# lmdu/pyfastx

Measured on NVIDIA H100. Metric: index_build_GBps, higher is better.
Workload: dtype u8

## Files before the change

### pyfastx_b200/csrc/fxg_scan.cu

```cuda
#include "fxg_common.cuh"
#include <stdlib.h>
#include <string.h>
#include <limits.h>

namespace fxg {

#ifndef FXG_MARK_MINB
#define FXG_MARK_MINB 6
#endif
constexpr int REGION   = 2048;
constexpr int SEGCAP   = 128;
constexpr int MARK_WARPS = 8;
constexpr int PS_THREADS = 256, PS_PER_THREAD = 16, PS_BLOCK = PS_THREADS * PS_PER_THREAD;
constexpr int64_t NOPOS = INT64_MIN / 4;
constexpr uint32_t E_POS = 0x07ffu, E_CR = 1u << 14, E_HDR = 1u << 15;
constexpr uint32_t FW_NF_SHIFT = 11, FW_NF = 3u << FW_NF_SHIFT, FW_GEN = 1u << 13;
constexpr int LF_MAX = 3, LF_STRIDE = 4;
constexpr uint32_t LF_HDR = 0, LF_LLEN = 1, LF_EVENT = 2, LF_CUT_UNKNOWN = 1u << 23;
constexpr uint32_t NAME_SCAN = 64;

struct __align__(16) FastaTmp {
    int64_t  boff;
    int64_t  lineidx;
    int64_t  llen;
// ... 503 lines not shown
        } else if (row < P.qrows_cap) {
            if (ph == 0) {
                int64_t l = len - 1;
                if (l > 0 && cr) --l;
                if (l < 0) l = 0;
                int64_t k = 0;
                if (s + 1 + l + 20 <= P.capacity) {
                    int which;
                    k = find_first_of2(file + s + 1, l, 0x20202020u, 0x00000000u, &which);
                    if (which == 2) k = l;
                } else {
                    for (; k < l; ++k) {
                        const uint8_t ch = file[s + 1 + k];
                        if (ch == 0) { k = l; break; }
                        if (ch == ' ') break;
                    }
                }
                *reinterpret_cast<int2 *>(&P.qrows[row].dlen) = make_int2((int)len, (int)k);
            } else if (ph == 3) {
                P.qrows[row].qoff = P.base_offset + s;
            }
        }
    }
}

template <int MODE>
__device__ __noinline__ Prev2 carry_walk(const ScanParams *Pg, int64_t r) {
    const ScanParams &P = *Pg;
    Prev2 cy;
    const int lane = threadIdx.x & 31;
    cy.pos1 = cy.pos0 = NOPOS; cy.h1 = cy.h0 = 0;
    int need = 2;
    auto push = [&](int64_t pos, uint32_t h) {
        if (need == 2) { cy.pos1 = pos; cy.h1 = h; } else { cy.pos0 = pos; cy.h0 = h; }
        --need;
    };
    int64_t q = r - 1;
    while (need > 0 && q >= 0) {
        const int64_t qq = q - lane;
        const uint32_t c = qq >= 0 ? (P.rc[qq].x & 0xffffu) : 0u;
        const uint32_t nz = __ballot_sync(0xffffffffu, c != 0);
        if (!nz) { q -= 32; continue; }
        const int f = __ffs(nz) - 1;
        q -= f;
        const int cq = (int)__shfl_sync(0xffffffffu, c, f);
        if (cq <= SEGCAP) {
            const uint32_t y = P.rc[q].y;
            push(q * REGION + (int64_t)(y & E_POS), MODE == 0 ? ((y >> 15) & 1u) : 0u);
            if (need > 0 && cq >= 2) push(q * REGION + (int64_t)((y >> 16) & E_POS), MODE == 0 ? (y >> 31) : 0u);
        } else {
            for (int64_t x = q * REGION + REGION - 1; x >= q * REGION && need > 0; --x)
                if (nl_at(P, x)) push(x, is_hdr_at<MODE>(P, x + 1));
        }
        q -= 1;
    }
    if (need > 0) push(-1, is_hdr_at<MODE>(P, 0));
    return cy;
}

template <int MODE>
__device__ __noinline__ unsigned long long dense_region(const ScanParams *Pg, int64_t first_line, int64_t r, Prev2 cy,
                                                        ulonglong2 exv) {
    const ScanParams &P = *Pg;
    unsigned long long my_size = 0;
    const int lane = threadIdx.x & 31;
    const uint8_t *file = P.file;
    const int64_t b0 = r * REGION + lane * 64;
    uint32_t c = 0, h = 0;
    Prev2 inc; inc.pos1 = inc.pos0 = NOPOS; inc.h1 = inc.h0 = 0;
    for (int i = 0; i < 64; ++i) {
        const int64_t x = b0 + i;
        if (nl_at(P, x)) {
            const uint32_t hh = is_hdr_at<MODE>(P, x + 1);
            ++c; h += hh;
            inc.pos0 = inc.pos1; inc.h0 = inc.h1; inc.pos1 = x; inc.h1 = hh;
        }
    }
    uint32_t ic = c, ih = h;
    uint32_t icnt = c > 2 ? 2 : c;
#pragma unroll
    for (int d = 1; d < 32; d <<= 1) {
        const uint32_t oc = __shfl_up_sync(0xffffffffu, ic, d), oh = __shfl_up_sync(0xffffffffu, ih, d);
        const int64_t op1 = shfl_up_i64(inc.pos1, d), op0 = shfl_up_i64(inc.pos0, d);
        const uint32_t oh1 = __shfl_up_sync(0xffffffffu, inc.h1, d), oh0 = __shfl_up_sync(0xffffffffu, inc.h0, d);
        const uint32_t ocnt = __shfl_up_sync(0xffffffffu, icnt, d);
        if (lane >= d) {
            ic += oc; ih += oh;
            if (icnt == 0) { inc.pos1 = op1; inc.h1 = oh1; inc.pos0 = op0; inc.h0 = oh0; icnt = ocnt; }
            else if (icnt == 1 && ocnt >= 1) { inc.pos0 = op1; inc.h0 = oh1; icnt = 2; }
        }
    }
    Prev2 pv;
    pv.pos1 = shfl_up_i64(inc.pos1, 1); pv.pos0 = shfl_up_i64(inc.pos0, 1);
    pv.h1 = __shfl_up_sync(0xffffffffu, inc.h1, 1); pv.h0 = __shfl_up_sync(0xffffffffu, inc.h0, 1);
    uint32_t pcnt = __shfl_up_sync(0xffffffffu, icnt, 1);
    if (lane == 0) pcnt = 0;
    if (pcnt == 0) pv = cy;
    else if (pcnt == 1) { pv.pos0 = cy.pos1; pv.h0 = cy.h1; }
    int64_t idx = (int64_t)exv.x + (ic - c);
    int64_t hcount = (int64_t)exv.y + (ih - h);
    for (int i = 0; i < 64 && c; ++i) {
        const int64_t x = b0 + i;
        if (!nl_at(P, x)) continue;
        const bool cr = x > 0 && file[x - 1] == '\r';
        do_line<MODE>(P, first_line, x, pv.pos1, pv.pos0, pv.h1 != 0, pv.h0 != 0, hcount, idx, cr, my_size);
        const uint32_t hh = is_hdr_at<MODE>(P, x + 1);
        hcount += hh; ++idx;
        pv.pos0 = pv.pos1; pv.h0 = pv.h1; pv.pos1 = x; pv.h1 = hh;
    }
    return my_size;
}

template <int MODE>
__device__ __forceinline__ void region_batches(const ScanParams &P, int64_t first_line, int64_t r, int nl, Prev2 cy, ulonglong2 X,
                                               uint32_t E0, uint32_t E1, unsigned long long &my_size) {
    const int lane = threadIdx.x & 31;
    const uint32_t lt_mask = (1u << lane) - 1u;
    const int64_t base = r * REGION;
    const uint16_t *sg = P.seg + r * SEGCAP;
    int64_t hrun = (int64_t)X.y;
    for (int k0 = 0; k0 < nl; k0 += 32) {
        const int k = k0 + lane;
        const bool valid = k < nl;
        uint32_t e = k0 == 0 ? E0 : (k0 == 32 ? E1 : (valid ? (uint32_t)sg[k] : 0u));
        if (!valid) e = 0;
        const uint32_t hb = __ballot_sync(0xffffffffu, (e & E_HDR) != 0);
        const uint32_t e1 = __shfl_up_sync(0xffffffffu, e, 1), e2 = __shfl_up_sync(0xffffffffu, e, 2);
        if (valid) {
            int64_t pm1, pm2;
            bool h1, h2;
            if (lane >= 1) { pm1 = base + (e1 & E_POS); h1 = (e1 & E_HDR) != 0; } else { pm1 = cy.pos1; h1 = cy.h1 != 0; }
            if (lane >= 2) { pm2 = base + (e2 & E_POS); h2 = (e2 & E_HDR) != 0; }
            else if (lane == 1) { pm2 = cy.pos1; h2 = cy.h1 != 0; }
            else { pm2 = cy.pos0; h2 = cy.h0 != 0; }
            do_line<MODE>(P, first_line, base + (e & E_POS), pm1, pm2, h1, h2, hrun + __popc(hb & lt_mask), (int64_t)X.x + k,
                          (e & E_CR) != 0, my_size);
        }
        const uint32_t l31 = __shfl_sync(0xffffffffu, e, 31), l30 = __shfl_sync(0xffffffffu, e, 30);
        cy.pos1 = base + (l31 & E_POS); cy.h1 = (l31 >> 15) & 1u;
        cy.pos0 = base + (l30 & E_POS); cy.h0 = (l30 >> 15) & 1u;
        hrun += __popc(hb);
    }
}

template <int MODE>
__device__ __noinline__ unsigned long long full_region(const ScanParams *Pg, int64_t first_line, int64_t r, ulonglong2 X) {
    const ScanParams &P = *Pg;
    unsigned long long my_size = 0;
    const int lane = threadIdx.x & 31;
    const int nl = (int)(P.rc[r].x & 0xffffu);
    if (nl == 0) return 0;
    Prev2 cy = carry_walk<MODE>(Pg, r);
    if (MODE != 0) cy.h1 = cy.h0 = 0;
    if (nl <= SEGCAP) region_batches<MODE>(P, first_line, r, nl, cy, X, P.seg[r * SEGCAP + lane], P.seg[r * SEGCAP + 32 + lane], my_size);
    else my_size += dense_region<MODE>(Pg, first_line, r, cy, X);
    return my_size;
}

constexpr int RG = 8;
constexpr int RWIN = RG + 2;
static_assert(RWIN * REGION <= 32768, "window positions must fit 15 bits");

__global__ void __launch_bounds__(MARK_WARPS * 32) fastq_records_kernel(const ScanParams Pin) {
    __shared__ uint16_t s_flat[MARK_WARPS][RWIN * SEGCAP];
    const ScanParams &P = Pin;
    const int64_t first_line = Pin.totals->first_line;
    const int lane = threadIdx.x & 31, warp = threadIdx.x >> 5;
    const int64_t r0 = ((int64_t)blockIdx.x * MARK_WARPS + warp) * RG;
    if (r0 >= P.nreg) return;
    unsigned long long my_size = 0;
    const uint8_t *file = P.file;

    const int64_t rl = r0 - 1 + lane;
    uint2 rec = make_uint2(0u, 0u);
    uint64_t exl = 0;
    if (lane <= RWIN && rl >= 0 && rl < P.nreg) { rec = P.rc[rl]; exl = P.ex[rl].x; }
    const uint32_t nll = rec.x & 0xffffu;
    const uint32_t densem = __ballot_sync(0xffffffffu, nll > (uint32_t)SEGCAP);
    if (densem & (((1u << RG) - 1u) << 1)) {
        for (int i = 0; i < RG; ++i)
            if (r0 + i < P.nreg) my_size += full_region<1>(P.self, first_line, r0 + i, P.ex[r0 + i]);
    } else {
        const uint64_t ex0 = (uint64_t)shfl_i64((int64_t)exl, 1);
        uint16_t *flat = s_flat[warp];
        int W = 0, Ls = 0;
        bool closed = false;
#pragma unroll
        for (int i = 0; i < RWIN; ++i) {
            const int nl = (int)__shfl_sync(0xffffffffu, nll, i + 1);
            if (nl > SEGCAP) closed = true;
            if (!closed) {
                const int k = 2 * lane;
                const uint32_t E2 = k < nl ? reinterpret_cast<const uint32_t *>(P.seg + (r0 + i) * SEGCAP)[lane] : 0u;
                const uint32_t e0 = E2 & 0xffffu, e1 = E2 >> 16;
                if (k < nl) flat[W + k] = (uint16_t)((i * REGION + (int)(e0 & E_POS)) | ((e0 & E_CR) ? 0x8000u : 0u));
                if (k + 1 < nl) flat[W + k + 1] = (uint16_t)((i * REGION + (int)(e1 & E_POS)) | ((e1 & E_CR) ? 0x8000u : 0u));
                if (nl > 64) {
                    const uint16_t *sg = P.seg + (r0 + i) * SEGCAP;
                    for (int kk = 64 + lane; kk < nl; kk += 32) {
                        const uint32_t e = sg[kk];
                        flat[W + kk] = (uint16_t)((i * REGION + (int)(e & E_POS)) | ((e & E_CR) ? 0x8000u : 0u));
                    }
                }
                W += nl;
            }
            if (i == RG - 1) Ls = W;
        }
        __syncwarp();
        int64_t carry;
        {
            const uint32_t pn = __shfl_sync(0xffffffffu, nll, 0), py = __shfl_sync(0xffffffffu, rec.y, 0);
            if (r0 == 0) carry = -1;
            else if (pn >= 1 && pn <= (uint32_t)SEGCAP) carry = (r0 - 1) * REGION + (int64_t)(py & E_POS);
            else carry = carry_walk<1>(P.self, r0).pos1;
        }
        const int64_t span_base = r0 * REGION;
        auto POS = [&](int f) -> int64_t { return f < 0 ? carry : span_base + (int64_t)(flat[f] & 0x7fffu); };
        auto CR = [&](int f) -> bool { return (flat[f] & 0x8000u) != 0; };
        const int64_t g0 = first_line + (int64_t)ex0;
        const int64_t row0 = first_line >> 2;
        int lead = (int)((4 - (g0 & 3)) & 3);
        if (lead > Ls) lead = Ls;
        if (lane < lead) {
            const int f = lane;
            const int64_t g = g0 + f;
            const int ph = (int)(g & 3);
            const int64_t row = (g >> 2) - row0;
            const int64_t pm1 = POS(f - 1), p = POS(f);
            if (ph == 1) {
                const int64_t len = p - pm1 - 1;
                const int64_t rlen = (len > 0 && CR(f)) ? len - 1 : len;
                my_size += (unsigned long long)rlen;
                if (row < P.qrows_cap) { P.qrows[row].soff = P.base_offset + pm1 + 1; P.qrows[row].rlen = rlen; }
            } else if (ph == 3) {
                if (row < P.qrows_cap) P.qrows[row].qoff = P.base_offset + pm1 + 1;
            }
        }
        for (int fb = lead; fb < Ls; fb += 128) {
            const int f = fb + 4 * lane;
            int64_t row = 0, soff = 0, rlen = 0, qoff = 0, len = 0, k = 0;
            bool have1 = false, have3 = false;
            const bool mine = f < Ls;
            if (mine) {
                row = ((g0 + f) >> 2) - row0;
                have1 = f + 1 < W; have3 = f + 3 < W;
                const int64_t pm1 = POS(f - 1), p0 = POS(f);
                len = p0 - pm1 - 1;
                int64_t l = len - 1;
                if (l > 0 && CR(f)) --l;
                if (l < 0) l = 0;
                const int64_t s = pm1 + 1;
                if (s + 1 + l + 20 <= P.capacity) {
                    int which;
                    k = find_first_of2(file + s + 1, l, 0x20202020u, 0x00000000u, &which);
                    if (which == 2) k = l;
                } else {
                    for (; k < l; ++k) {
                        const uint8_t ch = file[s + 1 + k];
                        if (ch == 0) { k = l; break; }
                        if (ch == ' ') break;
                    }
                }
                if (have1) {
                    const int64_t p1 = POS(f + 1);
                    const int64_t len1 = p1 - p0 - 1;
                    soff = P.base_offset + p0 + 1;
                    rlen = (len1 > 0 && CR(f + 1)) ? len1 - 1 : len1;
                    if (f + 1 < Ls) my_size += (unsigned long long)rlen;
                }
                if (have3) qoff = P.base_offset + POS(f + 2) + 1;
            }
            const bool full = mine && have3 && row < P.qrows_cap;
            const int other_full = __shfl_xor_sync(0xffffffffu, full ? 1 : 0, 1);
            const bool pair_full = full && other_full != 0;
            longlong2 a, b;
            a.x = soff; a.y = qoff;
            b.x = rlen; b.y = (long long)(((unsigned long long)(uint32_t)(int)k << 32) | (uint32_t)(int)len);
            const bool odd = (lane & 1) != 0;
            const longlong2 send = odd ? a : b;
            longlong2 recv;
            recv.x = shfl_i64(send.x, lane ^ 1);
            recv.y = shfl_i64(send.y, lane ^ 1);
            if (pair_full) {
                fxg_fastq_row *q0 = &P.qrows[odd ? row - 1 : row];
                reinterpret_cast<longlong2 *>(q0)[odd ? 1 : 0] = odd ? recv : a;
                reinterpret_cast<longlong2 *>(q0 + 1)[odd ? 1 : 0] = odd ? b : recv;
            } else if (mine && row < P.qrows_cap) {
                fxg_fastq_row *q = &P.qrows[row];
                if (have3) {
                    reinterpret_cast<longlong2 *>(q)[0] = a;
                    reinterpret_cast<longlong2 *>(q)[1] = b;
                } else {
                    *reinterpret_cast<int2 *>(&q->dlen) = make_int2((int)len, (int)k);
                    if (have1) { q->soff = soff; q->rlen = rlen; }
                }
            }
        }
    }
#pragma unroll
    for (int d = 16; d > 0; d >>= 1) my_size += (unsigned long long)shfl_down_i64((int64_t)my_size, d);
    if (lane == 0 && my_size) atomicAdd((unsigned long long *)&P.totals->sum_len, my_size);
}

constexpr int ROWS_THREADS = 1024, ROWS_PER_THREAD = PS_BLOCK / ROWS_THREADS;
static_assert(ROWS_PER_THREAD == 4, "one uint4 of first-entry words per thread");

__global__ void __launch_bounds__(ROWS_THREADS) fasta_rows_kernel(const ScanParams P) {
    __shared__ uint32_t s_a[ROWS_THREADS / 32], s_b[ROWS_THREADS / 32];
    const int lane = threadIdx.x & 31, warp = threadIdx.x >> 5;
    const int64_t r0 = (int64_t)blockIdx.x * PS_BLOCK + (int64_t)threadIdx.x * ROWS_PER_THREAD;
    const uint4 qa = reinterpret_cast<const uint4 *>(P.rc + r0)[0], qb = reinterpret_cast<const uint4 *>(P.rc + r0)[1];
    const uint4 fv = *reinterpret_cast<const uint4 *>(P.fw + r0);
    const uint2 rcv[ROWS_PER_THREAD] = {make_uint2(qa.x, qa.y), make_uint2(qa.z, qa.w), make_uint2(qb.x, qb.y), make_uint2(qb.z, qb.w)};
    const uint32_t fwv[ROWS_PER_THREAD] = {fv.x, fv.y, fv.z, fv.w};
    uint2 pv = r0 >= 1 ? P.rc[r0 - 1] : make_uint2(0u, 0u);
    uint32_t a = 0, b = 0;
#pragma unroll
    for (int i = 0; i < ROWS_PER_THREAD; ++i) { a += rcv[i].x & 0xffffu; b += rcv[i].x >> 16; }
    uint32_t ia = a, ib = b;
#pragma unroll
    for (int d = 1; d < 32; d <<= 1) {
        const uint32_t oa = __shfl_up_sync(0xffffffffu, ia, d), ob = __shfl_up_sync(0xffffffffu, ib, d);
        if (lane >= d) { ia += oa; ib += ob; }
    }
    const ulonglong2 bb = P.bs[blockIdx.x];
    if (lane == 31) { s_a[warp] = ia; s_b[warp] = ib; }
    __syncthreads();
    uint32_t wa = 0, wb = 0;
    for (int w = 0; w < warp; ++w) { wa += s_a[w]; wb += s_b[w]; }
    ulonglong2 X = make_ulonglong2(bb.x + wa + ia - a, bb.y + wb + ib - b);
    unsigned long long dummy = 0;
    bool any_general = false;
#pragma unroll
    for (int i = 0; i < ROWS_PER_THREAD; ++i) {
        const int64_t r = r0 + i, base = r * REGION;
        const uint32_t nl = rcv[i].x & 0xffffu, fw = fwv[i], pnl = pv.x & 0xffffu;
        const bool general = nl != 0 && (fw & FW_GEN) != 0;
        const bool walk = nl != 0 && !general && (r == 0 || pnl < 2u || pnl > (uint32_t)SEGCAP);
        Prev2 cy;
        cy.pos1 = base - REGION + (int64_t)(pv.y & E_POS); cy.h1 = (pv.y >> 15) & 1u;
        cy.pos0 = base - REGION + (int64_t)((pv.y >> 16) & E_POS); cy.h0 = pv.y >> 31;
        uint32_t wm = __ballot_sync(0xffffffffu, walk);
        while (wm) {
            const int f = __ffs(wm) - 1;
            wm &= wm - 1u;
            const Prev2 c = carry_walk<0>(P.self, shfl_i64(r, f));
            if (lane == f) cy = c;
        }
        if (general) *reinterpret_cast<ulonglong2 *>(P.lf + r * LF_STRIDE) = X;
        any_general |= general;
        if (nl != 0 && !general) {
            const uint32_t f0 = fw & 0xffffu, f1 = fw >> 16;
            const int64_t p0 = base + (int64_t)(f0 & E_POS);
            do_line<0>(P, 0, p0, cy.pos1, cy.pos0, cy.h1 != 0, cy.h0 != 0, (int64_t)X.y, (int64_t)X.x, false, dummy);
            if (nl >= 2u)
                do_line<0>(P, 0, base + (int64_t)(f1 & E_POS), p0, cy.pos1, (f0 & E_HDR) != 0, cy.h1 != 0,
                           (int64_t)X.y + ((f0 & E_HDR) ? 1 : 0), (int64_t)X.x + 1, false, dummy);
            const uint32_t nf = (fw & FW_NF) >> FW_NF_SHIFT;
            for (uint32_t j = 0; j < nf; ++j) {
                const uint2 lf = P.lf[r * LF_STRIDE + j];
                const int64_t slot = (int64_t)X.y + ((lf.x >> 16) & 31u), lineidx = (int64_t)X.x + ((lf.x >> 11) & 31u);
                if (slot >= P.tmp_cap) continue;
                const uint32_t kind = lf.x >> 21;
                if (kind == LF_HDR) {
                    const int64_t p = base + (int64_t)(lf.x & E_POS), dlen = lf.y & E_POS;
                    const int elen = 1 + (int)((lf.y >> 22) & 1u);
                    const int64_t nlen = (lf.y & LF_CUT_UNKNOWN) ? fasta_name_len(P, p - dlen - elen, dlen) : (int64_t)((lf.y >> 11) & E_POS);
                    fasta_header(P, slot, p, lineidx, dlen, nlen, elen);
                } else if (kind == LF_LLEN) {
                    P.tmp[slot].llen = lf.y;
                } else {
                    fasta_event(P, slot, lineidx, (int32_t)lf.y);
                }
            }
        }
        X.x += nl; X.y += rcv[i].x >> 16;
        pv = rcv[i];
    }
    const int block_general = __syncthreads_or(any_general ? 1 : 0);
    if (threadIdx.x == 0) P.gblk[blockIdx.x] = block_general ? 1u : 0u;
}

__global__ void __launch_bounds__(MARK_WARPS * 32) fasta_general_kernel(const ScanParams P) {
    __shared__ ulonglong2 s_x[MARK_WARPS][32];
    const int lane = threadIdx.x & 31, warp = threadIdx.x >> 5;
    const int64_t R0 = ((int64_t)blockIdx.x * MARK_WARPS + warp) * 32;
    if (R0 >= P.nreg) return;
    const int64_t r = R0 + lane;
    if (!P.gblk[R0 / PS_BLOCK]) return;
    const bool general = r < P.nreg && (P.fw[r] & FW_GEN) != 0;
    if (general) s_x[warp][lane] = *reinterpret_cast<const ulonglong2 *>(P.lf + r * LF_STRIDE);
    uint32_t gm = __ballot_sync(0xffffffffu, general);
    while (gm) {
        const int f = __ffs(gm) - 1;
        gm &= gm - 1u;
        full_region<0>(P.self, 0, R0 + f, s_x[warp][f]);
    }
}

__global__ void __launch_bounds__(256) fasta_finalize_kernel(const FastaTmp *tmp, int64_t tmp_cap, int64_t rows_cap,
                                                             int64_t base_offset, ScanTotals *tot, fxg_fasta_row *rows) {
    int64_t nrows = (int64_t)tot->hdr;
    if (nrows > rows_cap || nrows + 1 > tmp_cap) nrows = 0;
    unsigned long long slen_acc = 0;
    const int64_t stride = (int64_t)gridDim.x * blockDim.x;
    for (int64_t r = (int64_t)blockIdx.x * blockDim.x + threadIdx.x; r < nrows; r += stride) {
        const FastaTmp t = tmp[r + 1];
        int64_t next_h, next_line;
        if (r + 1 < nrows) {
            const FastaTmp nx = tmp[r + 2];
            next_h = nx.boff - (1 + nx.dlen + (int64_t)nx.elen);
            next_line = nx.lineidx;
        } else {
            next_h = base_offset + tot->n_eff;
            next_line = (int64_t)tot->nl;
        }
        const int64_t blen = next_h - t.boff;
        const int64_t nlines = next_line - t.lineidx - 1;
        const int64_t slen = blen - nlines * (int64_t)t.elen;
        int norm;
        if (t.D == 0) norm = 1;
        else if (t.D == 1) norm = ((int64_t)t.evmax == t.lineidx + nlines) ? 1 : 0;
        else if (t.D == 2) norm = ((t.evmax - (~t.evminc) == 1) && t.S == 0) ? 1 : 0;
        else norm = 0;
        fxg_fasta_row o;
        o.boff = t.boff; o.blen = blen; o.slen = slen; o.llen = t.llen;
        o.dlen = t.dlen; o.nlen = t.nlen; o.elen = (uint8_t)t.elen; o.norm = (uint8_t)norm;
        for (int i = 0; i < 6; ++i) o.pad[i] = 0;
        o.pad[0] = (t.D == 0 || (t.D == 1 && (int64_t)t.evmax == t.lineidx + nlines && (int64_t)t.S < 0)) ? 1 : 0;
        rows[r] = o;
        slen_acc += (unsigned long long)slen;
    }
#pragma unroll
    for (int d = 16; d > 0; d >>= 1) slen_acc += (unsigned long long)shfl_down_i64((int64_t)slen_acc, d);
    if ((threadIdx.x & 31) == 0 && slen_acc) atomicAdd((unsigned long long *)&tot->sum_len, slen_acc);
    if (blockIdx.x == 0 && threadIdx.x == 0) {
        const FastaTmp l = tmp[0];
        tot->lead_llen = l.llen;
        if (nrows > 0) {
            const FastaTmp f = tmp[1];
            tot->lead_lines = f.lineidx;
            tot->lead_bytes = f.boff - base_offset - (1 + f.dlen + (int64_t)f.elen);
        }
    }
}

__global__ void __launch_bounds__(32) edge_kernel(const ScanParams P, int mode, fxg_shard_info *info) {
    const int lane = threadIdx.x;
    int found = 0;
    int64_t pos[3] = {0, 0, 0};
    for (int64_t r0 = 0; r0 < P.nreg && found < 3; r0 += 32) {
        const int64_t r = r0 + lane;
        const uint32_t c = r < P.nreg ? (P.rc[r].x & 0xffffu) : 0u;
        uint32_t nz = __ballot_sync(0xffffffffu, c != 0);
        while (nz && found < 3) {
            const int fl = __ffs(nz) - 1;
            nz &= nz - 1;
            const int64_t q = r0 + fl;
            for (int64_t x0 = q * REGION; x0 < q * REGION + REGION && found < 3; x0 += 512) {
                const int64_t x = x0 + lane * 16;
                uint32_t m = 0;
                if (x + 16 <= P.n) {
                    const uint4 v = *reinterpret_cast<const uint4 *>(P.file + x);
                    const uint32_t w[4] = {v.x, v.y, v.z, v.w};
#pragma unroll
                    for (int i = 0; i < 16; ++i) m |= (((w[i >> 2] >> (8 * (i & 3))) & 0xffu) == '\n' ? 1u : 0u) << i;
                } else {
                    for (int i = 0; i < 16; ++i) m |= (nl_at(P, x + i) ? 1u : 0u) << i;
                }
                uint32_t any = __ballot_sync(0xffffffffu, m != 0);
                while (any && found < 3) {
                    const int fl2 = __ffs(any) - 1;
                    any &= any - 1u;
                    uint32_t mm = __shfl_sync(0xffffffffu, m, fl2);
                    while (mm && found < 3) { pos[found++] = x0 + fl2 * 16 + (__ffs(mm) - 1); mm &= mm - 1u; }
                }
            }
        }
    }
    if (lane == 0) {
        const ScanTotals t = *P.totals;
        fxg_shard_info o;
        o.n_rows = mode == 0 ? (int64_t)t.hdr : 0;
        o.n_lines = (int64_t)t.nl;
        o.bytes = P.n;
        o.base_offset = P.base_offset;
        o.end_position = t.n_eff;
        o.edge_n = found;
        int64_t start = 0;
        for (int j = 0; j < 3; ++j) {
            o.edge_off[j] = 0; o.edge_len[j] = 0;
            if (j < found) {
                const int64_t p = pos[j];
                const bool cr = p > start && p - 1 < P.n && P.file[p - 1] == '\r';
                o.edge_off[j] = P.base_offset + start;
                o.edge_len[j] = p - start - (cr ? 1 : 0);
                start = p + 1;
            }
        }
        for (int j = 0; j < 4; ++j) o.reserved[j] = 0;
        *info = o;
    }
}

__global__ void shard_prefix_kernel(const fxg_shard_info *all, int nranks, int rank, int mode, ScanTotals *tot) {
    if (threadIdx.x != 0 || blockIdx.x != 0) return;
    int64_t F = 0, T = 0;
    for (int p = 0; p < nranks; ++p) {
        const int64_t nlp = all[p].n_lines;
        if (p < rank) F += nlp;
        T += nlp;
    }
    if (mode == 0) F = 0;
    tot->first_line = F;
    tot->total_lines = T;
    const int64_t nl = (int64_t)tot->nl;
    tot->nrows = mode == 0 ? (int64_t)tot->hdr : (F + nl + 3) / 4 - F / 4;
    tot->sum_len = 0;
}

__global__ void __launch_bounds__(256) clear_kernel(const ScanParams P, int mode, int64_t tmp_slots) {
    const int64_t nrows = P.totals->nrows;
    const int64_t stride = (int64_t)gridDim.x * blockDim.x;
    const int64_t t0 = (int64_t)blockIdx.x * blockDim.x + threadIdx.x;
    if (mode == 0) {
        int64_t slots = nrows + 2;
        if (slots > tmp_slots) slots = tmp_slots;
        uint4 *p = reinterpret_cast<uint4 *>(P.tmp);
        for (int64_t i = t0; i < slots * 4; i += stride) p[i] = make_uint4(0u, 0u, 0u, 0u);
    } else if (t0 < 4) {
        const int64_t row = t0 < 2 ? 0 : nrows - 1;
        if (row >= 0 && row < P.qrows_cap) reinterpret_cast<uint4 *>(P.qrows + row)[t0 & 1] = make_uint4(0u, 0u, 0u, 0u);
    }
}

__global__ void fastq_stitch_kernel(const ScanParams P, const fxg_shard_info *all, int nranks, int rank) {
    if (threadIdx.x != 0 || blockIdx.x != 0) return;
    ScanTotals *tot = P.totals;
    const int64_t F = tot->first_line, n = (int64_t)tot->nl, T = tot->total_lines;
    const int64_t first_read = (F + 3) / 4;
    int64_t last_read = n > 0 ? (F + n - 1) / 4 : first_read - 1;
    if (last_read > T / 4 - 1) last_read = T / 4 - 1;
    const int64_t owned = last_read >= first_read ? last_read - first_read + 1 : 0;
    tot->row0 = first_read - F / 4;
    tot->n_owned = owned;
    if (owned == 0) return;
    const int64_t row = last_read - F / 4;
    if (row >= P.qrows_cap) return;
    for (int ph = 1; ph <= 3; ph += 2) {
        const int64_t g = 4 * last_read + ph;
        if (g < F + n) continue;
        int64_t Fp = F + n;
        for (int p = rank + 1; p < nranks; ++p) {
            const int64_t np = all[p].n_lines;
            if (g < Fp + np) {
                const int64_t j = g - Fp;
                if (j < all[p].edge_n) {
                    if (ph == 1) { P.qrows[row].soff = all[p].edge_off[j]; P.qrows[row].rlen = all[p].edge_len[j]; }
                    else P.qrows[row].qoff = all[p].edge_off[j];
                }
                break;
            }
            Fp += np;
        }
    }
}

__global__ void __launch_bounds__(256) split_point_kernel(const uint8_t *file, int64_t n, int64_t from, int want_header,
                                                          long long *out) {
    __shared__ long long s_best;
    if (threadIdx.x == 0) s_best = LLONG_MAX;
    __syncthreads();
    if (from <= 0) {
        if (!want_header || (n > 0 && file[0] == '>')) { if (threadIdx.x == 0) *out = 0; return; }
        from = 1;
    }
    for (int64_t c0 = from - 1; c0 < n; c0 += 256 * 16) {
        const int64_t a = c0 + threadIdx.x * 16;
        long long mine = LLONG_MAX;
        for (int i = 0; i < 16; ++i) {
            const int64_t x = a + i;
            if (x < n && file[x] == '\n' && (!want_header || (x + 1 < n && file[x + 1] == '>'))) { mine = x + 1; break; }
        }
        if (mine != LLONG_MAX) atomicMin(&s_best, mine);
        __syncthreads();
        if (s_best != LLONG_MAX) break;
        __syncthreads();
    }
    if (threadIdx.x == 0) *out = s_best == LLONG_MAX ? n : s_best;
}

}

using namespace fxg;

static int64_t guess_rows(int mode, int64_t n) { return (mode == 0 ? n / 1024 : n / 200) + 4096; }

static int scan_params(fxg_ctx *ctx, const fxg_file *f, int mode, int64_t base_offset, int flags, bool reserve,
                       ScanParams *out, int64_t *tmp_slots) {
    const int64_t n = f->size;
    const int64_t nreg = (n + 1 + REGION - 1) / REGION;
    const int64_t nb = (nreg + PS_BLOCK - 1) / PS_BLOCK;
    const int64_t nreg_pad = nb * PS_BLOCK;
    const size_t off_bs = fxg_round_up((int64_t)nreg_pad * 8, 256);
    const size_t off_x = off_bs + fxg_round_up(nb * (int64_t)sizeof(ulonglong2), 256);
    const size_t off_gb = off_x + fxg_round_up(nreg_pad * (int64_t)sizeof(uint32_t), 256);
    const size_t off_lf = off_gb + fxg_round_up(nb * (int64_t)sizeof(uint32_t), 256);
    const size_t tile_bytes = mode == 0 ? off_lf + (size_t)nreg * LF_STRIDE * sizeof(uint2) : off_x + (size_t)nreg * sizeof(ulonglong2);
    int rc;
    if (reserve) {
        if ((rc = ctx->counters.reserve(1024))) return rc;
        if ((rc = ctx->tile_desc.reserve(tile_bytes))) return rc;
        if ((rc = ctx->seg.reserve((size_t)nreg * SEGCAP * sizeof(uint16_t)))) return rc;
        const int64_t want = guess_rows(mode, n);
        if (mode == 0) {
            if (ctx->row_tmp.cap < (size_t)(want + 2) * sizeof(FastaTmp) && (rc = ctx->row_tmp.reserve((size_t)(want + 2) * sizeof(FastaTmp)))) return rc;
            if (ctx->rows.cap < (size_t)(want + 1) * sizeof(fxg_fasta_row) && (rc = ctx->rows.reserve((size_t)(want + 1) * sizeof(fxg_fasta_row)))) return rc;
        } else if (ctx->rows.cap < (size_t)(want + 2) * sizeof(fxg_fastq_row)) {
            if ((rc = ctx->rows.reserve((size_t)(want + 2) * sizeof(fxg_fastq_row)))) return rc;
        }
    }
    ScanParams P;
    memset(&P, 0, sizeof(P));
    P.file = f->d; P.n = n; P.capacity = f->capacity & ~(int64_t)15; P.nreg = nreg;
    P.base_offset = base_offset; P.first_line = 0; P.flags = flags;
    P.rc = (uint2 *)ctx->tile_desc.ptr;
    P.bs = (ulonglong2 *)((uint8_t *)ctx->tile_desc.ptr + off_bs);
    if (mode == 0) {
        P.fw = (uint32_t *)((uint8_t *)ctx->tile_desc.ptr + off_x);
        P.gblk = (uint32_t *)((uint8_t *)ctx->tile_desc.ptr + off_gb);
        P.lf = (uint2 *)((uint8_t *)ctx->tile_desc.ptr + off_lf);
    } else {
        P.ex = (ulonglong2 *)((uint8_t *)ctx->tile_desc.ptr + off_x);
    }
    P.seg = (uint16_t *)ctx->seg.ptr;
    P.totals = (ScanTotals *)((uint8_t *)ctx->counters.ptr + 64);
    *tmp_slots = 0;
    if (mode == 0) {
        *tmp_slots = (int64_t)(ctx->row_tmp.cap / sizeof(FastaTmp));
        P.tmp = (FastaTmp *)ctx->row_tmp.ptr;
        P.tmp_cap = *tmp_slots - 1;
    } else {
        P.qrows = (fxg_fastq_row *)ctx->rows.ptr;
        P.qrows_cap = (int64_t)(ctx->rows.cap / sizeof(fxg_fastq_row));
    }
    *out = P;
    return FXG_OK;
}

static fxg_shard_info *own_info(fxg_ctx *ctx) { return (fxg_shard_info *)((uint8_t *)ctx->counters.ptr + 256); }

extern "C" int fxg_scan_begin(fxg_ctx *ctx, const fxg_file *f, int mode, int64_t base_offset, int flags,
                              fxg_shard_info *d_info_out) {
    FXG_CHECK_ARG(ctx && f && (mode == 0 || mode == 1), "null ctx/file or bad mode");
    FXG_LOCK(ctx);
    FXG_CUDA(cudaSetDevice(ctx->device));
    ctx->run.active = false;
    ScanParams P;
    int64_t tmp_slots;
    int rc = scan_params(ctx, f, mode, base_offset, flags, true, &P, &tmp_slots);
    if (rc) return rc;
    const int64_t n = f->size, nreg = P.nreg;
    const int64_t nb = (nreg + PS_BLOCK - 1) / PS_BLOCK, nreg_pad = nb * PS_BLOCK;
    FXG_CUDA(cudaMemsetAsync(ctx->counters.ptr, 0, 1024, ctx->stream));
    if (nreg_pad > nreg) FXG_CUDA(cudaMemsetAsync(P.rc + nreg, 0, (size_t)(nreg_pad - nreg) * 8, ctx->stream));
    const unsigned grid = (unsigned)((nreg + MARK_WARPS - 1) / MARK_WARPS);
    {
        FxgProfScope prof(ctx, FXG_PROF_SCAN);
        if (mode == 0) mark_kernel<0, 1><<<grid, MARK_WARPS * 32, 0, ctx->stream>>>(P);
        else mark_kernel<1, 2><<<grid, MARK_WARPS * 32, 0, ctx->stream>>>(P);
    }
    FXG_CUDA(cudaGetLastError());
    {
        FxgProfScope prof(ctx, FXG_PROF_PREFIX, mode == 0 ? 3 : 4);
        prefix_reduce_kernel<<<(unsigned)nb, PS_THREADS, 0, ctx->stream>>>(P.rc, P.bs);
        prefix_blocks_kernel<<<1, 1024, 0, ctx->stream>>>(P.bs, nb, P.file, n, mode, P.totals);
        if (mode == 1) prefix_expand_kernel<<<(unsigned)nb, PS_THREADS, 0, ctx->stream>>>(P.rc, P.bs, P.ex, nreg);
        edge_kernel<<<1, 32, 0, ctx->stream>>>(P, mode, own_info(ctx));
    }
    FXG_CUDA(cudaGetLastError());
    if (d_info_out)
        FXG_CUDA(cudaMemcpyAsync(d_info_out, own_info(ctx), sizeof(fxg_shard_info), cudaMemcpyDeviceToDevice, ctx->stream));
    ctx->run.active = true; ctx->run.mode = mode; ctx->run.flags = flags; ctx->run.file = f; ctx->run.base_offset = base_offset;
    return FXG_OK;
}

static int launch_phase_b(fxg_ctx *ctx, const ScanParams &P0, int mode, int64_t tmp_slots, const fxg_shard_info *d_all,
                          int nranks, int rank) {
    int rc0 = ctx->params.reserve(512);
    if (rc0) return rc0;
    if (!ctx->h_counters) FXG_CUDA(cudaHostAlloc(&ctx->h_counters, 8192, cudaHostAllocDefault));
    ScanParams P = P0;
    P.self = (const ScanParams *)ctx->params.ptr;
    static_assert(sizeof(ScanParams) <= 512, "ScanParams staging");
    memcpy((uint8_t *)ctx->h_counters + 4096, &P, sizeof(P));
    FXG_CUDA(cudaMemcpyAsync(ctx->params.ptr, (uint8_t *)ctx->h_counters + 4096, sizeof(P), cudaMemcpyHostToDevice, ctx->stream));
    const int64_t nreg = P.nreg;
    {
        FxgProfScope prof(ctx, FXG_PROF_LINES, mode == 0 ? 4 : 3);
        shard_prefix_kernel<<<1, 32, 0, ctx->stream>>>(d_all, nranks, rank, mode, P.totals);
        clear_kernel<<<ctx->sm_count * 4, 256, 0, ctx->stream>>>(P, mode, tmp_slots);
        if (mode == 0) {
            const int64_t nb = (nreg + PS_BLOCK - 1) / PS_BLOCK;
            fasta_rows_kernel<<<(unsigned)nb, ROWS_THREADS, 0, ctx->stream>>>(P);
            fasta_general_kernel<<<(unsigned)((nreg + MARK_WARPS * 32 - 1) / (MARK_WARPS * 32)), MARK_WARPS * 32, 0, ctx->stream>>>(P);
        } else {
            const unsigned lgrid = (unsigned)((nreg + MARK_WARPS * RG - 1) / (MARK_WARPS * RG));
            fastq_records_kernel<<<lgrid, MARK_WARPS * 32, 0, ctx->stream>>>(P);
        }
    }
    FXG_CUDA(cudaGetLastError());
    {
        FxgProfScope prof(ctx, FXG_PROF_FINALIZE);
        if (mode == 0)
            fasta_finalize_kernel<<<ctx->sm_count * 4, 256, 0, ctx->stream>>>(
                P.tmp, P.tmp_cap, (int64_t)(ctx->rows.cap / sizeof(fxg_fasta_row)), P.base_offset, P.totals,
                (fxg_fasta_row *)ctx->rows.ptr);
        else
            fastq_stitch_kernel<<<1, 32, 0, ctx->stream>>>(P, d_all, nranks, rank);
    }
    FXG_CUDA(cudaGetLastError());
    return FXG_OK;
}

extern "C" int fxg_scan_finish(fxg_ctx *ctx, const fxg_shard_info *d_all, int nranks, int rank, void **d_rows_out,
                               fxg_scan_stats *stats, fxg_shard_info *all_host) {
    FXG_CHECK_ARG(ctx && stats && nranks >= 1 && rank >= 0 && rank < nranks, "bad arguments");
    FXG_LOCK(ctx);
    FXG_CHECK_ARG(ctx->run.active, "fxg_scan_finish without fxg_scan_begin");
    FXG_CUDA(cudaSetDevice(ctx->device));
    ctx->run.active = false;
    const int mode = ctx->run.mode;
    const fxg_file *f = ctx->run.file;
    if (!d_all) { FXG_CHECK_ARG(nranks == 1, "d_all == NULL with more than one rank"); d_all = own_info(ctx); }
    memset(stats, 0, sizeof(*stats));
    if (d_rows_out) *d_rows_out = nullptr;
    if (!ctx->h_counters) FXG_CUDA(cudaHostAlloc(&ctx->h_counters, 8192, cudaHostAllocDefault));
    FXG_CHECK_ARG((size_t)nranks * sizeof(fxg_shard_info) + 256 <= 4096 || !all_host, "too many ranks for all_host");
    ScanTotals *ht = (ScanTotals *)ctx->h_counters;
    fxg_shard_info *hall = (fxg_shard_info *)((uint8_t *)ctx->h_counters + 256);
    for (int attempt = 0; attempt < 2; ++attempt) {
        ScanParams P;
        int64_t tmp_slots;
        int rc = scan_params(ctx, f, mode, ctx->run.base_offset, ctx->run.flags, false, &P, &tmp_slots);
        if (rc) return rc;
        if ((rc = launch_phase_b(ctx, P, mode, tmp_slots, d_all, nranks, rank))) return rc;
        FXG_CUDA(cudaMemcpyAsync(ht, P.totals, sizeof(ScanTotals), cudaMemcpyDeviceToHost, ctx->stream));
        if (all_host)
            FXG_CUDA(cudaMemcpyAsync(hall, d_all, (size_t)nranks * sizeof(fxg_shard_info), cudaMemcpyDeviceToHost, ctx->stream));
        FXG_CUDA(cudaStreamSynchronize(ctx->stream));
        bool fits;
        if (mode == 0) fits = ht->nrows + 2 <= tmp_slots && (size_t)(ht->nrows + 1) * sizeof(fxg_fasta_row) <= ctx->rows.cap;
        else fits = ht->nrows <= P.qrows_cap;
        if (fits) break;
        if (attempt == 1) { fxg_set_error("row buffers still too small after regrowing"); return FXG_ENOMEM; }
        if (mode == 0) {
            if ((rc = ctx->row_tmp.reserve((size_t)(ht->nrows + 2) * sizeof(FastaTmp)))) return rc;
            if ((rc = ctx->rows.reserve((size_t)(ht->nrows + 1) * sizeof(fxg_fasta_row)))) return rc;
        } else if ((rc = ctx->rows.reserve((size_t)(ht->nrows + 2) * sizeof(fxg_fastq_row)))) return rc;
    }
    stats->n_lines = (int64_t)ht->nl;
    stats->end_position = ht->n_eff;
    stats->total_len = (int64_t)ht->sum_len;
    if (mode == 0) {
        stats->n_rows = ht->nrows;
        stats->lead_llen = ht->lead_llen;
        if (ht->nrows > 0) { stats->lead_lines = ht->lead_lines; stats->lead_bytes = ht->lead_bytes; }
        else { stats->lead_lines = (int64_t)ht->nl; stats->lead_bytes = f->size; }
        if (d_rows_out) *d_rows_out = ctx->rows.ptr;
    } else {
        stats->n_rows = ht->n_owned;
        stats->lead_lines = ht->first_line;
        stats->reserved = ht->total_lines;
        if (d_rows_out) *d_rows_out = (fxg_fastq_row *)ctx->rows.ptr + ht->row0;
    }
    if (all_host) memcpy(all_host, hall, (size_t)nranks * sizeof(fxg_shard_info));
    return FXG_OK;
}

extern "C" int fxg_scan_sharded(fxg_ctx *ctx, fxg_comm *comm, const fxg_file *f, int mode, int64_t base_offset, int flags,
                                void **d_rows_out, fxg_scan_stats *stats, fxg_shard_info *all_host) {
    FXG_CHECK_ARG(ctx && f && stats, "null ctx/file/stats");
    FXG_LOCK(ctx);
    const int nranks = comm ? fxg_comm_nranks(comm) : 1, rank = comm ? fxg_comm_rank(comm) : 0;
    int rc = ctx->misc.reserve((size_t)nranks * sizeof(fxg_shard_info) + 256);
    if (rc) return rc;
    fxg_shard_info *d_all = (fxg_shard_info *)ctx->misc.ptr;
    if ((rc = fxg_scan_begin(ctx, f, mode, base_offset, flags, nullptr))) return rc;
    if ((rc = fxg_shard_exchange(ctx, comm, own_info(ctx), d_all, sizeof(fxg_shard_info)))) return rc;
    if ((rc = fxg_scan_finish(ctx, d_all, nranks, rank, d_rows_out, stats, all_host))) return rc;
    return comm ? fxg_comm_check(comm) : FXG_OK;
}

extern "C" int fxg_fasta_scan(fxg_ctx *ctx, const fxg_file *f, int64_t base_offset, int flags,
                              fxg_fasta_row **d_rows_out, fxg_scan_stats *stats) {
    FXG_CHECK_ARG(ctx && f && stats, "null ctx/file/stats");
    FXG_LOCK(ctx);
    int rc = fxg_scan_begin(ctx, f, 0, base_offset, flags, nullptr);
    if (rc) return rc;
    return fxg_scan_finish(ctx, nullptr, 1, 0, (void **)d_rows_out, stats, nullptr);
}

extern "C" int fxg_fastq_scan(fxg_ctx *ctx, const fxg_file *f, int64_t base_offset,
                              fxg_fastq_row **d_rows_out, fxg_scan_stats *stats) {
    FXG_CHECK_ARG(ctx && f && stats, "null ctx/file/stats");
    FXG_LOCK(ctx);
    int rc = fxg_scan_begin(ctx, f, 1, base_offset, 0, nullptr);
    if (rc) return rc;
    return fxg_scan_finish(ctx, nullptr, 1, 0, (void **)d_rows_out, stats, nullptr);
}

extern "C" int fxg_split_point_dev(fxg_ctx *ctx, const fxg_file *f, int64_t from, int want_header, int64_t *pos) {
    FXG_CHECK_ARG(ctx && f && pos && from >= 0, "bad arguments");
    FXG_LOCK(ctx);
    FXG_CUDA(cudaSetDevice(ctx->device));
    if (from >= f->size) { *pos = f->size; return FXG_OK; }
    int rc;
    if ((rc = ctx->counters.reserve(1024))) return rc;
    long long *d = (long long *)((uint8_t *)ctx->counters.ptr + 512);
    ctx->launches += 1;
    split_point_kernel<<<1, 256, 0, ctx->stream>>>(f->d, f->size, from, want_header, d);
    FXG_CUDA(cudaGetLastError());
    long long h = 0;
    FXG_CUDA(cudaMemcpyAsync(&h, d, 8, cudaMemcpyDeviceToHost, ctx->stream));
    FXG_CUDA(cudaStreamSynchronize(ctx->stream));
    *pos = (int64_t)h;
    return FXG_OK;
}
```

Baseline: 2512.

## Split fasta_rows_kernel into smaller CTAs with in-block prefix recompute

Shrinks fasta_rows_kernel from 1024 threads covering a whole prefix block to 256-thread CTAs, each covering a quarter of it, and launches four times as many CTAs. Each CTA recomputes the partial newline and header counts of the earlier CTAs in its prefix block by rereading their row counters and warp-reducing them. The general-block flag array is now indexed per small CTA, and its allocation is resized to match. The goal is better occupancy and more parallelism when there are few prefix blocks, at the cost of redundant counter reads that grow for later CTAs in each block.

```diff
diff --git a/pyfastx_b200/csrc/fxg_scan.cu b/pyfastx_b200/csrc/fxg_scan.cu
--- a/pyfastx_b200/csrc/fxg_scan.cu
+++ b/pyfastx_b200/csrc/fxg_scan.cu
@@ -829,13 +829,23 @@
     if (lane == 0 && my_size) atomicAdd((unsigned long long *)&P.totals->sum_len, my_size);
 }
 
-constexpr int ROWS_THREADS = 1024, ROWS_PER_THREAD = PS_BLOCK / ROWS_THREADS;
-static_assert(ROWS_PER_THREAD == 4, "one uint4 of first-entry words per thread");
+constexpr int ROWS_THREADS = 256, ROWS_PER_THREAD = 4, ROWS_REGIONS = ROWS_THREADS * ROWS_PER_THREAD;
+static_assert(PS_BLOCK % ROWS_REGIONS == 0, "whole CTAs per prefix block");
 
 __global__ void __launch_bounds__(ROWS_THREADS) fasta_rows_kernel(const ScanParams P) {
-    __shared__ uint32_t s_a[ROWS_THREADS / 32], s_b[ROWS_THREADS / 32];
+    constexpr int NW = ROWS_THREADS / 32;
+    __shared__ uint32_t s_a[NW], s_b[NW], s_pa[NW], s_pb[NW];
     const int lane = threadIdx.x & 31, warp = threadIdx.x >> 5;
-    const int64_t r0 = (int64_t)blockIdx.x * PS_BLOCK + (int64_t)threadIdx.x * ROWS_PER_THREAD;
+    const int64_t c0 = (int64_t)blockIdx.x * ROWS_REGIONS, blk = c0 / PS_BLOCK;
+    const int64_t r0 = c0 + (int64_t)threadIdx.x * ROWS_PER_THREAD;
+    uint32_t pa = 0, pb = 0;
+    for (int64_t x = blk * PS_BLOCK + (int64_t)threadIdx.x * ROWS_PER_THREAD; x < c0; x += ROWS_REGIONS) {
+        const uint4 u = reinterpret_cast<const uint4 *>(P.rc + x)[0], w = reinterpret_cast<const uint4 *>(P.rc + x)[1];
+        pa += (u.x & 0xffffu) + (u.z & 0xffffu) + (w.x & 0xffffu) + (w.z & 0xffffu);
+        pb += (u.x >> 16) + (u.z >> 16) + (w.x >> 16) + (w.z >> 16);
+    }
+    pa = __reduce_add_sync(0xffffffffu, pa);
+    pb = __reduce_add_sync(0xffffffffu, pb);
     const uint4 qa = reinterpret_cast<const uint4 *>(P.rc + r0)[0], qb = reinterpret_cast<const uint4 *>(P.rc + r0)[1];
     const uint4 fv = *reinterpret_cast<const uint4 *>(P.fw + r0);
     const uint2 rcv[ROWS_PER_THREAD] = {make_uint2(qa.x, qa.y), make_uint2(qa.z, qa.w), make_uint2(qb.x, qb.y), make_uint2(qb.z, qb.w)};
@@ -850,11 +860,15 @@
         const uint32_t oa = __shfl_up_sync(0xffffffffu, ia, d), ob = __shfl_up_sync(0xffffffffu, ib, d);
         if (lane >= d) { ia += oa; ib += ob; }
     }
-    const ulonglong2 bb = P.bs[blockIdx.x];
-    if (lane == 31) { s_a[warp] = ia; s_b[warp] = ib; }
+    const ulonglong2 bb = P.bs[blk];
+    if (lane == 31) { s_a[warp] = ia; s_b[warp] = ib; s_pa[warp] = pa; s_pb[warp] = pb; }
     __syncthreads();
     uint32_t wa = 0, wb = 0;
-    for (int w = 0; w < warp; ++w) { wa += s_a[w]; wb += s_b[w]; }
+#pragma unroll
+    for (int w = 0; w < NW; ++w) {
+        wa += s_pa[w] + (w < warp ? s_a[w] : 0u);
+        wb += s_pb[w] + (w < warp ? s_b[w] : 0u);
+    }
     ulonglong2 X = make_ulonglong2(bb.x + wa + ia - a, bb.y + wb + ib - b);
     unsigned long long dummy = 0;
     bool any_general = false;
@@ -914,7 +928,7 @@
     const int64_t R0 = ((int64_t)blockIdx.x * MARK_WARPS + warp) * 32;
     if (R0 >= P.nreg) return;
     const int64_t r = R0 + lane;
-    if (!P.gblk[R0 / PS_BLOCK]) return;
+    if (!P.gblk[R0 / ROWS_REGIONS]) return;
     const bool general = r < P.nreg && (P.fw[r] & FW_GEN) != 0;
     if (general) s_x[warp][lane] = *reinterpret_cast<const ulonglong2 *>(P.lf + r * LF_STRIDE);
     uint32_t gm = __ballot_sync(0xffffffffu, general);
@@ -1132,7 +1146,7 @@
     const size_t off_bs = fxg_round_up((int64_t)nreg_pad * 8, 256);
     const size_t off_x = off_bs + fxg_round_up(nb * (int64_t)sizeof(ulonglong2), 256);
     const size_t off_gb = off_x + fxg_round_up(nreg_pad * (int64_t)sizeof(uint32_t), 256);
-    const size_t off_lf = off_gb + fxg_round_up(nb * (int64_t)sizeof(uint32_t), 256);
+    const size_t off_lf = off_gb + fxg_round_up(nreg_pad / ROWS_REGIONS * (int64_t)sizeof(uint32_t), 256);
     const size_t tile_bytes = mode == 0 ? off_lf + (size_t)nreg * LF_STRIDE * sizeof(uint2) : off_x + (size_t)nreg * sizeof(ulonglong2);
     int rc;
     if (reserve) {
@@ -1229,7 +1243,7 @@
         clear_kernel<<<ctx->sm_count * 4, 256, 0, ctx->stream>>>(P, mode, tmp_slots);
         if (mode == 0) {
             const int64_t nb = (nreg + PS_BLOCK - 1) / PS_BLOCK;
-            fasta_rows_kernel<<<(unsigned)nb, ROWS_THREADS, 0, ctx->stream>>>(P);
+            fasta_rows_kernel<<<(unsigned)(nb * (PS_BLOCK / ROWS_REGIONS)), ROWS_THREADS, 0, ctx->stream>>>(P);
             fasta_general_kernel<<<(unsigned)((nreg + MARK_WARPS * 32 - 1) / (MARK_WARPS * 32)), MARK_WARPS * 32, 0, ctx->stream>>>(P);
         } else {
             const unsigned lgrid = (unsigned)((nreg + MARK_WARPS * RG - 1) / (MARK_WARPS * RG));
```

Result: no change. 2503 (median of 6 runs) (-0.4%).
